# DeepMETv2/DeepMETv2

Measured on AMD Instinct MI355X. Metric: events/sec (4.5k PF cands, k=16), higher is better.
Workload: dtype f32

## Files before the change

deepmetv2_amd/csrc/knn.hip:

```cpp
#include <stdlib.h>

#include "common.h"
#include "knn_common.h"
#include "knn_key64.h"
#include "nls_body.h"

namespace dmet {
namespace {

constexpr int kTileC = 32;
constexpr int kQMax = 8;
constexpr int kMaxSplit = 8;
constexpr int kWavesPerGroup = 4;

#define DMET_PKSUB_LO " op_sel:[0,0] op_sel_hi:[0,1] neg_lo:[0,1] neg_hi:[0,1]\n\t"
#define DMET_PKSUB_HI " op_sel:[1,0] op_sel_hi:[1,1] neg_lo:[0,1] neg_hi:[0,1]\n\t"
__device__ __forceinline__ void pk_dist_step4(f2 &accA, f2 &accB, f2 vxy, f2 vzw, f2 wxy, f2 wzw, f2 q0, f2 q1, f2 q2,
                                              f2 q3)
{
    f2 t0, t1, t2, t3;
    asm("v_pk_add_f32 %[t0], %[vxy], %[q0]" DMET_PKSUB_LO
        "v_pk_add_f32 %[t1], %[wxy], %[q0]" DMET_PKSUB_LO
        "v_pk_add_f32 %[t2], %[vxy], %[q1]" DMET_PKSUB_HI
        "v_pk_add_f32 %[t3], %[wxy], %[q1]" DMET_PKSUB_HI
// ... 105 lines not shown
        for (int p = 0; p < KP; p += 4) {
            *reinterpret_cast<float4 *>(ld + p) = make_float4(d[p], d[p + 1], d[p + 2], d[p + 3]);
            *reinterpret_cast<int4 *>(lj + p) = make_int4(j[p], j[p + 1], j[p + 2], j[p + 3]);
        }
    }
    return d[KP - 1];
}

#ifdef DMET_KNN_STAMP
__device__ unsigned long long g_knn_stamps[1 << 16][4];
#endif

#ifndef DMET_F2_MIN_NODES
#define DMET_F2_MIN_NODES 800
#endif
constexpr int kF2MinNodes = DMET_F2_MIN_NODES;
constexpr int kFilterMaxSplit = 2;
#ifndef DMET_F2_SPLIT_MIN_NODES
#define DMET_F2_SPLIT_MIN_NODES 2560
#endif
constexpr int kF2SplitMinNodes = DMET_F2_SPLIT_MIN_NODES;
constexpr int kF2MaxNodes = 65536;

struct KnnPlan {
    int total_tiles;
    int n_full;
    int split;
    int form1_events;
};

struct KnnArgs {
    const float *x;
    const int64_t *ptr;
    int B;
    int64_t N;
    int D, k;
    int32_t *nbr;
    float *dist;
    uint16_t *nbr16;
    float *wsd;
    int32_t *wsj;
    const KnnPlan *plan;
    const int32_t *order;
    const int32_t *tile_ptr;
    float *psd;
    int32_t *psj;
    const int32_t *flags;
    int flag_min;
    const int32_t *any;
    const int32_t *qlist;
    const int32_t *pos_of;
    int requery_groups;
    int requery_tile_queries;
};

__device__ __forceinline__ uint16_t local_id16(int32_t j, int ev_lo)
{
    return (uint16_t)(j >= 0 ? (unsigned)(j - ev_lo) : 0xFFFFu);
}

constexpr int kMaxSortedEvents = 4096;

struct KnnPlanOut {
    int tile_queries, simds, max_split;
    int32_t *order, *pos_of, *tile_ptr;
    KnnPlan *plan;
};

__device__ __forceinline__ int xcd_dealt_position(int rank, int B)
{
    if (B < 4 * kNumXcd) return rank;
    const int c = rank % (2 * kNumXcd), g = rank / (2 * kNumXcd);
    const int bin = c < kNumXcd ? c : 2 * kNumXcd - 1 - c;
    const int idx = 2 * g + (c >= kNumXcd ? 1 : 0);
    const int rem = B % (2 * kNumXcd), full = B / (2 * kNumXcd);
    int start = 0;
    for (int b = 0; b < bin; ++b)
        start += 2 * full + (b < min(rem, kNumXcd) ? 1 : 0) + ((rem > kNumXcd && b > 2 * kNumXcd - 1 - rem) ? 1 : 0);
    return start + idx;
}

template <bool XY = false>
__device__ __forceinline__ void knn_plan_body(const int64_t *__restrict__ ptr, int B, const KnnPlanOut &o,
                                              const int64_t *__restrict__ cptr = nullptr)
{
    const int tile_queries = o.tile_queries, simds = o.simds, max_split = o.max_split;
    int32_t *__restrict__ order = o.order, *__restrict__ pos_of = o.pos_of, *__restrict__ tile_ptr = o.tile_ptr;
    KnnPlan *__restrict__ plan = o.plan;
    __shared__ int part[256];
    const int tid = threadIdx.x;
    if (B <= kMaxSortedEvents) {
        for (int b = tid; b < B; b += 256) {
            const int64_t nb = ptr[b + 1] - ptr[b];
            int rank = 0;
            if constexpr (XY) {
                const int64_t xb = nb > 0 ? cptr[b + 1] - cptr[b] : -1;
                for (int c = 0; c < B; ++c) {
                    const int64_t nc = ptr[c + 1] - ptr[c];
                    const int64_t xc = nc > 0 ? cptr[c + 1] - cptr[c] : -1;
                    rank += (xc > xb || (xc == xb && (nc > nb || (nc == nb && c < b)))) ? 1 : 0;
                }
            } else {
                for (int c = 0; c < B; ++c) {
                    const int64_t nc = ptr[c + 1] - ptr[c];
                    rank += (nc > nb || (nc == nb && c < b)) ? 1 : 0;
                }
// ... 110 lines not shown
    int lo = 0, hi = B;
    while (hi - lo > 1) {
        const int mid = (lo + hi) >> 1;
        if (tile_ptr[mid] <= t) lo = mid; else hi = mid;
    }
    return lo;
}

template <int DP, bool EXACT_D, int NLD>
__device__ __forceinline__ void load_tile(float4 (&pf)[NLD], const float *__restrict__ x, int D, int c0, int cntc,
                                          int lane)
{
    const float inf = __builtin_inff();
    if (EXACT_D) {
        const float4 *g = reinterpret_cast<const float4 *>(x + (int64_t)c0 * DP);
        const int n4 = cntc * (DP / 4);
#pragma unroll
        for (int m = 0; m < NLD; ++m) {
            const int idx = lane + m * kWave;
            pf[m] = (idx < n4) ? g[idx] : make_float4(inf, inf, inf, inf);
        }
    } else {
#pragma unroll
        for (int m = 0; m < NLD; ++m) {
            float v[4];
#pragma unroll
            for (int e = 0; e < 4; ++e) {
                const int flat = (lane + m * kWave) * 4 + e;
                const int c = flat / DP, dd = flat - c * DP;
                v[e] = (c < cntc) ? ((dd < D) ? x[(int64_t)(c0 + c) * D + dd] : 0.0f) : inf;
            }
            pf[m] = make_float4(v[0], v[1], v[2], v[3]);
        }
    }
}

__device__ __forceinline__ float chain_dist32(const float *__restrict__ xj, const float (&q)[32])
{
    const float4 *g = reinterpret_cast<const float4 *>(xj);
    float acc = 0.0f;
#pragma unroll
    for (int c = 0; c < 8; ++c) {
        const float4 v = g[c];
        float df;
        df = v.x - q[4 * c + 0]; acc = __builtin_fmaf(df, df, acc);
        df = v.y - q[4 * c + 1]; acc = __builtin_fmaf(df, df, acc);
        df = v.z - q[4 * c + 2]; acc = __builtin_fmaf(df, df, acc);
        df = v.w - q[4 * c + 3]; acc = __builtin_fmaf(df, df, acc);
    }
    return acc;
}

constexpr int kRequeryMax = 8;
constexpr int kRequeryGroups = 512;

__device__ __forceinline__ unsigned long long requery_word(float d, int j)
{
    return d < kKnnSentinel ? (((unsigned long long)__float_as_uint(d) << 32) | (unsigned)j) : ~0ull;
}

__device__ __forceinline__ void knn_requery_body(const KnnArgs &a, float *__restrict__ cache, const int cache_floats,
                                                 unsigned long long *__restrict__ red, const int group, const int ngroups)
{
    const int tid = threadIdx.x, wv = tid >> 6, lane = tid & 63;
    const int64_t nf64 = *a.any;
    const int nflag = (int)(nf64 < a.N ? nf64 : a.N);
    const int k = a.k;
    for (int it = group; it < nflag; it += ngroups) {
        const int q = a.qlist[it];
        int lo = 0, hi = a.B;
        while (hi - lo > 1) {
            const int mid = (lo + hi) >> 1;
            if (a.ptr[mid] <= q) lo = mid; else hi = mid;
        }
        const int ev = lo;
        const int ev_lo = (int)a.ptr[ev], ev_hi = (int)a.ptr[ev + 1];
        const int n = ev_hi - ev_lo;
        const int xt = a.tile_ptr[a.pos_of[ev]] + (q - ev_lo) / a.requery_tile_queries;
        if (a.flags[xt] > kRequeryMax) continue;
        const bool cached = n <= cache_floats;
        float qrow[32];
        {
            const float4 *g = reinterpret_cast<const float4 *>(a.x + (int64_t)q * 32);
#pragma unroll
            for (int c = 0; c < 8; ++c) {
                const float4 v = g[c];
                qrow[4 * c] = v.x; qrow[4 * c + 1] = v.y; qrow[4 * c + 2] = v.z; qrow[4 * c + 3] = v.w;
            }
        }
        __syncthreads();
        if (cached) {
            for (int j0 = tid; j0 < n; j0 += 4 * 256) {
                float4 r[4][8];
#pragma unroll
                for (int u = 0; u < 4; ++u) {
                    const float4 *g = reinterpret_cast<const float4 *>(a.x + (int64_t)(ev_lo + min(j0 + 256 * u, n - 1)) * 32);
#pragma unroll
                    for (int c = 0; c < 8; ++c) r[u][c] = g[c];
                }
#pragma unroll
                for (int u = 0; u < 4; ++u) {
                    float dc = 0.0f;
#pragma unroll
                    for (int c = 0; c < 8; ++c) {
                        float df;
                        df = r[u][c].x - qrow[4 * c + 0]; dc = __builtin_fmaf(df, df, dc);
                        df = r[u][c].y - qrow[4 * c + 1]; dc = __builtin_fmaf(df, df, dc);
                        df = r[u][c].z - qrow[4 * c + 2]; dc = __builtin_fmaf(df, df, dc);
                        df = r[u][c].w - qrow[4 * c + 3]; dc = __builtin_fmaf(df, df, dc);
                    }
                    if (j0 + 256 * u < n) cache[j0 + 256 * u] = dc;
                }
            }
            __syncthreads();
        }
        unsigned long long last = 0ull;
        bool first = true;
        for (int r = 0; r < k; ++r) {
            unsigned long long best = ~0ull;
            for (int j = tid; j < n; j += 256) {
                const float d = cached ? cache[j] : chain_dist32(a.x + (int64_t)(ev_lo + j) * 32, qrow);
                const unsigned long long w = requery_word(d, ev_lo + j);
                if ((first || w > last) && w < best) best = w;
            }
#pragma unroll
            for (int off = 32; off > 0; off >>= 1) {
                const unsigned long long o = __shfl_xor(best, off, 64);
                if (o < best) best = o;
            }
            if (lane == 0) red[wv] = best;
            __syncthreads();
            best = red[0];
#pragma unroll
            for (int w = 1; w < 4; ++w) if (red[w] < best) best = red[w];
            __syncthreads();
            const bool found = best != ~0ull;
            if (tid == 0) {
                const int bj = found ? (int)(unsigned)best : -1;
                a.nbr[(int64_t)q * k + r] = bj;
                if (a.nbr16) a.nbr16[(int64_t)q * k + r] = local_id16(bj, ev_lo);
                a.dist[(int64_t)q * k + r] = found ? __uint_as_float((unsigned)(best >> 32)) : kKnnSentinel;
            }
            if (!found) {
                if (tid == 0)
                    for (int rr = r + 1; rr < k; ++rr) {
                        a.nbr[(int64_t)q * k + rr] = -1;
                        a.dist[(int64_t)q * k + rr] = kKnnSentinel;
                        if (a.nbr16) a.nbr16[(int64_t)q * k + rr] = 0xFFFFu;
                    }
                break;
            }
            last = best;
            first = false;
        }
    }
}

template <int DP, int KP, int TQ, bool EXACT_D, typename... Per>
__global__ __launch_bounds__(kWave * kWavesPerGroup, 3) void knn_kernel(const KnnArgs a, Per... per_arg)
{
    constexpr bool PER = pack_has<RadPeriod, Per...>, XY = pack_has<KnnQuerySet, Per...>;
    static_assert(!PER || TQ == 2, "the periodic sweep is the packed two-query form (D <= 8)");
    const RadPeriod per = rad_periods(per_arg...);
    __shared__ KnnShared<DP, TQ> sh_all[kWavesPerGroup];
    const int wv_ = __builtin_amdgcn_readfirstlane(threadIdx.x >> 6);
    KnnShared<DP, TQ> &sh = sh_all[wv_];
    int first_group = 0;
    if constexpr (DP == 32 && !XY) {
        if (a.qlist) {
            if (a.any && *a.any == 0) return;
            if ((int)blockIdx.x < a.requery_groups) {
                constexpr int kFloats = (int)((sizeof(sh_all) - 64) / sizeof(float));
                knn_requery_body(a, reinterpret_cast<float *>(sh_all), kFloats,
                                 reinterpret_cast<unsigned long long *>(reinterpret_cast<char *>(sh_all) + sizeof(sh_all) - 64),
                                 (int)blockIdx.x, a.requery_groups);
                return;
            }
            first_group = a.requery_groups;
        }
    }
    const int item = ((int)blockIdx.x - first_group) * kWavesPerGroup + wv_;
    const int lane = threadIdx.x & 63;
#ifdef DMET_KNN_STAMP
    if (lane == 0 && item < (1 << 16)) {
        g_knn_stamps[item][0] = __builtin_amdgcn_s_memrealtime();
        unsigned hwid, xcc;
        asm volatile("s_getreg_b32 %0, hwreg(HW_REG_HW_ID)" : "=s"(hwid));
        asm volatile("s_getreg_b32 %0, hwreg(HW_REG_XCC_ID)" : "=s"(xcc));
        g_knn_stamps[item][2] = hwid;
        g_knn_stamps[item][3] = xcc;
        g_knn_stamps[item][1] = 0;
    }
#endif
    const float *__restrict__ x = a.x;
    const int64_t *__restrict__ ptr = a.ptr;
    const KnnQuerySet qs = query_set(a.x, a.ptr, per_arg...);
    const float *__restrict__ qx = qs.qx;
    const int64_t *__restrict__ qptr = qs.qptr;
    const int D = a.D;
    constexpr int QT = kWave * TQ;

    const int n_full = a.plan->n_full, split = a.plan->split, total = a.plan->total_tiles;
    int tile = item, sub = 0, nsub = 1;
    if (item >= n_full && !a.flags) {
        const int r = item - n_full;
        tile = n_full + r / split;
        sub = r % split;
        nsub = split;
    }
    if (tile >= total) return;
    if (a.any && *a.any == 0) return;
    if (a.flags && a.flags[tile] < a.flag_min) return;
    const int pos = find_tile_event(a.tile_ptr, a.B, tile);
    const int ev = a.order[pos];
    const int ev_lo = (int)qptr[ev], ev_hi = (int)qptr[ev + 1];
    const int q_first = ev_lo + (tile - a.tile_ptr[pos]) * QT;

    int clo = XY ? (int)ptr[ev] : ev_lo, chi = XY ? (int)ptr[ev + 1] : ev_hi;
    if (nsub > 1) {
        const int chunk = (((chi - clo) + nsub - 1) / nsub + 1) & ~1;
        clo = min(chi, clo + sub * chunk);
        chi = min(chi, clo + chunk);
    }

    int qi[TQ];
    bool valid[TQ];
    float tau[TQ];
    int cnt[TQ];
    float *ld[TQ];
    int32_t *lj[TQ];
    f2 q2[(TQ == 2) ? DP : 1];
    float q1[(TQ == 1) ? DP : 1];
#pragma unroll
    for (int t = 0; t < TQ; ++t) {
        qi[t] = q_first + t * kWave + lane;
// ... 78 lines not shown
                    df = v.z - q1[4 * c4 + 2]; accA = __builtin_fmaf(df, df, accA);
                    df = w.z - q1[4 * c4 + 2]; accB = __builtin_fmaf(df, df, accB);
                    df = v.w - q1[4 * c4 + 3]; accA = __builtin_fmaf(df, df, accA);
                    df = w.w - q1[4 * c4 + 3]; accB = __builtin_fmaf(df, df, accB);
                }
                dA[0] = accA; dB[0] = accB;
            }
#pragma unroll
            for (int t = 0; t < TQ; ++t) {
#pragma unroll
                for (int u = 0; u < 2; ++u) {
                    const float dj = u ? dB[t] : dA[t];
                    bool pass = dj < tau[t];
#ifdef DMET_KNN_NOSELECT
                    pass = pass && (dj < -1.0f);
#endif
                    if (pass) {
                        sh.queue[t][cnt[t]][lane] = make_uint2(__float_as_uint(dj), (unsigned)(c0 + cc + u));
                        cnt[t]++;
                    }
                }
                if (__any(cnt[t] > kQMax - 2)) {
                    tau[t] = drain_queue<KP>(sh.queue[t], lane, cnt[t], (fresh >> t) & 1u, valid[t], ld[t], lj[t]);
                    if (!valid[t]) tau[t] = -1.0f;
                    cnt[t] = 0;
                    fresh &= ~(1u << t);
                }
            }
        }
    }
#ifdef DMET_KNN_STAMP
    if (lane == 0 && item < (1 << 16)) g_knn_stamps[item][1] = __builtin_amdgcn_s_memrealtime();
#endif
#pragma unroll
    for (int t = 0; t < TQ; ++t) {
        (void)drain_queue<KP>(sh.queue[t], lane, cnt[t], (fresh >> t) & 1u, valid[t], ld[t], lj[t]);
        if (valid[t] && nsub == 1) {
            const int64_t qq = qi[t];
            if (a.k == KP) {
#pragma unroll
                for (int p = 0; p < KP; p += 4) {
                    *reinterpret_cast<float4 *>(a.dist + qq * KP + p) = *reinterpret_cast<const float4 *>(ld[t] + p);
                    *reinterpret_cast<int4 *>(a.nbr + qq * KP + p) = *reinterpret_cast<const int4 *>(lj[t] + p);
                }
            } else {
                for (int p = 0; p < a.k; ++p) {
                    a.dist[qq * a.k + p] = ld[t][p];
                    a.nbr[qq * a.k + p] = lj[t][p];
                }
            }
            if (a.nbr16)
                for (int p = 0; p < a.k; ++p) a.nbr16[qq * a.k + p] = local_id16(lj[t][p], ev_lo);
        }
    }
}

template <int KP, typename... Qs>
__global__ __launch_bounds__(256) void knn_merge_kernel(const KnnArgs a, int tile_queries, Qs... qs_arg)
{
    if (a.any && *a.any == 0) return;
    const int n_full = a.plan->n_full, split = a.plan->split, total = a.plan->total_tiles;
    if (split <= 1) return;
    const int64_t slot = (int64_t)blockIdx.x * blockDim.x + threadIdx.x;
    const int tile = n_full + (int)(slot / tile_queries);
    if (tile >= total) return;
    if (a.flags && a.flags[tile] < a.flag_min) return;
    const int pos = find_tile_event(a.tile_ptr, a.B, tile);
    const int ev = a.order[pos];
    const int64_t *__restrict__ qptr = query_set(a.x, a.ptr, qs_arg...).qptr;
    const int64_t qi = qptr[ev] + (int64_t)(tile - a.tile_ptr[pos]) * tile_queries + (slot % tile_queries);
    if (qi >= qptr[ev + 1]) return;
    const float *pd = a.psd + slot * split * KP;
    const int32_t *pj = a.psj + slot * split * KP;
    int head[kMaxSplit];
#pragma unroll
    for (int s = 0; s < kMaxSplit; ++s) head[s] = 0;
    for (int p = 0; p < a.k; ++p) {
        float bd = kKnnSentinel;
        int32_t bj = -1;
        int bs = -1;
#pragma unroll
        for (int s = 0; s < kMaxSplit; ++s) {
            if (s < split && head[s] < KP) {
                const float d = pd[s * KP + head[s]];
                const int32_t j = pj[s * KP + head[s]];
                if (j >= 0 && (bs < 0 || d < bd || (d == bd && j < bj))) { bd = d; bj = j; bs = s; }
            }
        }
#pragma unroll
        for (int s = 0; s < kMaxSplit; ++s) head[s] += (s == bs) ? 1 : 0;
        a.dist[qi * a.k + p] = bd;
        a.nbr[qi * a.k + p] = bj;
        if (a.nbr16) a.nbr16[qi * a.k + p] = local_id16(bj, (int)a.ptr[ev]);
    }
}

#include "knn_filter.h"

int num_simds()
{
    static int cached = 0;
    if (cached == 0) {
        int dev = 0, cus = 0;
        if (hipGetDevice(&dev) == hipSuccess &&
            hipDeviceGetAttribute(&cus, hipDeviceAttributeMultiprocessorCount, dev) == hipSuccess && cus > 0)
            cached = cus * 4;
// ... 78 lines not shown
    w.pos_of = reinterpret_cast<int32_t *>(take(sizeof(int32_t) * ((size_t)B + 1)));
    w.tile_ptr = reinterpret_cast<int32_t *>(take(sizeof(int32_t) * ((size_t)B + 1)));
    w.wsd = reinterpret_cast<float *>(take(sizeof(float) * (size_t)N * KP));
    w.wsj = reinterpret_cast<int32_t *>(take(sizeof(int32_t) * (size_t)N * KP));
    w.psd = reinterpret_cast<float *>(take(sizeof(float) * ps_elems));
    w.psj = reinterpret_cast<int32_t *>(take(sizeof(int32_t) * ps_elems));
    if (!exact_only) {
        w.fplan = reinterpret_cast<KnnPlan *>(take(sizeof(KnnPlan)));
        w.forder = reinterpret_cast<int32_t *>(take(sizeof(int32_t) * ((size_t)B + 1)));
        w.fpos_of = reinterpret_cast<int32_t *>(take(sizeof(int32_t) * ((size_t)B + 1)));
        w.ftile_ptr = reinterpret_cast<int32_t *>(take(sizeof(int32_t) * ((size_t)B + 1)));
        w.nrm = reinterpret_cast<float *>(take(sizeof(float) * (size_t)N));
        w.nrec = (N >> 5) + B + 1;
        w.rec = reinterpret_cast<uint8_t *>(take((size_t)w.nrec * kRecBytesMax));
        w.zero_bytes = sizeof(int32_t) * ((size_t)exact_tiles_max(N, B) + 4) + (size_t)N;
        w.flags = reinterpret_cast<int32_t *>(take(w.zero_bytes));
        w.any = w.flags + exact_tiles_max(N, B);
        w.qflag = reinterpret_cast<uint8_t *>(w.any + 4);
        w.qlist = reinterpret_cast<int32_t *>(take(sizeof(int32_t) * (size_t)N));
    }
    w.bytes = (size_t)(p - reinterpret_cast<uintptr_t>(ws));
    return w;
}

inline int filter_mode()
{
    const char *e = getenv("DMET_KNN_PATH");
    if (e && strcmp(e, "exact") == 0) return 0;
#if defined(DMET_KNN_EXPERIMENT) || defined(DMET_FILTER_ABL) || defined(DMET_F2_ABL) || defined(DMET_F2_SAMEREC)
    if (e && strcmp(e, "filter_only") == 0) return 2;
#endif
    return 1;
}

inline int filter_form2()
{
    const char *e = getenv("DMET_KNN_FILTER");
    return (e && strcmp(e, "1") == 0) ? 0 : 1;
}

constexpr float kF2CutScale = 1.25f;
inline float knn_cut_scale()
{
    const char *e = getenv("DMET_KNN_CUT");
    if (!e || !*e) return kF2CutScale;
    if (strcmp(e, "0") == 0 || strcmp(e, "off") == 0) return -1.0f;
    char *end = nullptr;
    const float v = strtof(e, &end);
    return (end != e && *end == '\0' && v >= 0.0f && v <= 1e6f) ? v : kF2CutScale;
}

inline int knn_run_cut() { return env_is("DMET_KNN_RUNCUT", "0") ? 0 : 1; }

template <int KF, int NH = 1>
int launch_filter(const KnnFilterArgs &f, const KnnWorkspace &w, int simds, const KnnPlanOut &px, const KnnPlanOut &pf,
                  hipStream_t st, const KnnRider *rider, const BnAffine *affine)
{
    const int slots = simds * kF2WavesPerSimd;
    if (affine) {
        if constexpr (NH == 1)
            hipLaunchKernelGGL((knn_prep_kernel<1, true>), dim3((unsigned)((w.nrec * kWave + 255) / 256 + 2)), dim3(256), 0, st, f.x,
                               f.ptr, f.B, f.N, w.nrm, w.rec, w.nrec, reinterpret_cast<uint32_t *>(w.flags), w.zero_bytes, px,
                               pf, f.form2, *affine, 0);
    } else {
        hipLaunchKernelGGL((knn_prep_kernel<NH>), dim3((unsigned)((w.nrec * kWave + 255) / 256 + 2)), dim3(256), 0, st, f.x,
                           f.ptr, f.B, f.N, w.nrm, w.rec, w.nrec, reinterpret_cast<uint32_t *>(w.flags), w.zero_bytes, px, pf,
                           f.form2, BnAffine{}, 0);
    }
    DMET_LAUNCH_CHECK("knn_prep_kernel");
    const int64_t ftiles_max = (f.N + kFQ - 1) / kFQ + f.B;
    const int64_t fblocks = (ftiles_max + slots + kWavesPerGroup - 1) / kWavesPerGroup;
    if (f.form2) {
        KnnFilterArgs fr = f;
        int64_t grid = fblocks;
        if (rider) {
            fr.rW = rider->W; fr.rb = rider->b; fr.rP = rider->P; fr.rQ = rider->Q; fr.r_sliced = rider->sliced;
            fr.first_rider = (int)fblocks;
            grid = fblocks + rider_groups();
        }
        hipLaunchKernelGGL((knn_filter12_kernel<KF, NH>), dim3((unsigned)grid), dim3(kWave * kWavesPerGroup), 0, st, fr);
        DMET_LAUNCH_CHECK("knn_filter12_kernel");
    } else {
        if constexpr (NH == 1) hipLaunchKernelGGL((knn_filter_kernel<KF>), dim3((unsigned)fblocks), dim3(kWave * kWavesPerGroup), 0, st, f);
        DMET_LAUNCH_CHECK("knn_filter_kernel");
    }
    constexpr int kRerankQpb = 4 * (kWave / filter_list_len(KF));
    constexpr int kRerankParts = (kFQ + kRerankQpb - 1) / kRerankQpb;
    const int64_t tail_max = ftiles_max < slots ? ftiles_max : slots;
    if constexpr (NH == 1) {
        if (f.no_rerank) return 0;
        hipLaunchKernelGGL((knn_rerank_kernel<KF>), dim3((unsigned)(tail_max * kRerankParts)), dim3(256), 0, st, f);
        DMET_LAUNCH_CHECK("knn_rerank_kernel");
    }
    return 0;
}

template <int DP, int KP, int TQ>
void launch_sweep(int64_t blocks, unsigned dyn, hipStream_t st, const KnnArgs &a, bool exact_d, const RadPeriod *per,
                  const KnnQuerySet *qs)
{
    const dim3 grid((unsigned)blocks), block(kWave * kWavesPerGroup);
    with_pack<DP <= 8, true>(per, qs, [&](auto... pack) {
        if (exact_d) hipLaunchKernelGGL((knn_kernel<DP, KP, TQ, true, decltype(pack)...>), grid, block, dyn, st, a, pack...);
        else hipLaunchKernelGGL((knn_kernel<DP, KP, TQ, false, decltype(pack)...>), grid, block, dyn, st, a, pack...);
    });
}

template <int KP>
void launch_merge(int64_t slots, hipStream_t st, const KnnArgs &a, int tile_queries, const KnnQuerySet *qs)
{
    with_pack<false, true>(nullptr, qs, [&](auto... pack) {
        hipLaunchKernelGGL((knn_merge_kernel<KP, decltype(pack)...>), dim3((unsigned)((slots + 255) / 256)), dim3(256), 0, st, a,
                           tile_queries, pack...);
    });
}

template <int DP, int KP>
KnnOutcome launch_knn(const KnnBuild &r, const KnnWorkspace &w)
{
    KnnOutcome done;
    constexpr int TQ = (DP <= 32) ? 2 : 1;
    constexpr int QT = kWave * TQ;
    const KnnQuerySet *qs = r.qs.qx ? &r.qs : nullptr;
    int simds = num_simds();
    if (simds > kMaxSimds) simds = kMaxSimds;
    bool use_filter = false;
    if constexpr ((DP == 32 || DP == 64) && KP <= 32)
        use_filter = !qs && r.D == DP && r.k <= 20 && aligned16(r.x) && filter_mode() != 0 && (DP == 32 || filter_form2());
    constexpr int NH = DP == 64 ? 2 : 1;
    const int slots = simds * kF2WavesPerSimd;
    const KnnPlanOut px{QT, simds, kMaxSplit, w.order, w.pos_of, w.tile_ptr, w.plan};
    const KnnPlanOut pf{kFQ, slots, kFilterMaxSplit, w.forder, w.fpos_of, w.ftile_ptr, w.fplan};
    if (qs) {
        hipLaunchKernelGGL(knn_plan_xy_kernel, dim3(1), dim3(256), 0, r.st, qs->qptr, r.ptr, r.B, px);
        DMET_LAUNCH_CHECK("knn_plan_xy_kernel");
    } else if (!use_filter) {
        hipLaunchKernelGGL(knn_plan_kernel, dim3(1), dim3(256), 0, r.st, r.ptr, r.B, px, pf);
        DMET_LAUNCH_CHECK("knn_plan_kernel");
    }
    KnnArgs a{r.x, r.ptr, r.B, r.N, r.D, r.k, r.nbr, r.dist, r.nbr16, w.wsd, w.wsj, w.plan, w.order, w.tile_ptr, w.psd, w.psj,
              nullptr, 0, nullptr, nullptr, nullptr, 0, QT};
    if (!qs && !use_filter && hipMemsetAsync(w.flags, 0, w.zero_bytes, r.st) != hipSuccess)
        return hip_fail(hipGetLastError(), "hipMemsetAsync");

    if (use_filter) {
        KnnFilterArgs f{r.x, r.ptr, r.B, r.N, r.k, w.nrm, w.rec, w.fplan, w.forder, w.fpos_of, w.ftile_ptr,
                        w.psd, w.psj, r.nbr, r.dist, r.nbr16, w.flags, w.any, w.qflag, w.qlist, w.tile_ptr, QT, filter_form2(),
                        NH == 1 ? 1.0f : 1.5f, nullptr, nullptr, nullptr, nullptr, 0, 0,
                        (aligned16(r.nbr) && aligned16(r.dist) && aligned16(r.nbr16) && !env_is("DMET_KNN_EMIT", "lanes")) ? 1 : 0, 0,
                        knn_cut_scale(), w.any + 1, knn_run_cut()};
        f.no_rerank = (f.form2 && r.hint.min_nodes >= kF2MinNodes && r.hint.max_nodes >= r.hint.min_nodes &&
                       r.hint.max_nodes <= kF2MaxNodes) ? 1 : 0;
        const BnAffine *affine = (NH == 1 && r.affine.raw) ? &r.affine : nullptr;
        const KnnRider *rider = (NH == 1 && f.form2 && r.rider.P) ? &r.rider : nullptr;
        int rc = 0;
        if constexpr (DP == 32 || DP == 64) {
            if constexpr (KP == 8) rc = launch_filter<8, NH>(f, w, simds, px, pf, r.st, rider, affine);
            else if constexpr (KP == 16) rc = launch_filter<16, NH>(f, w, simds, px, pf, r.st, rider, affine);
            else if constexpr (KP == 32) rc = launch_filter<20, NH>(f, w, simds, px, pf, r.st, rider, affine);
        }
        if (rc) return rc;
        done.affine_done = affine != nullptr;
        done.rider_done = rider != nullptr;
        if (filter_mode() == 2) return done;
        a.flags = w.flags;
        a.any = w.any;
        if constexpr (NH == 1) {
            a.qlist = w.qlist;
            a.pos_of = w.pos_of;
            a.requery_groups = kRequeryGroups;
            a.flag_min = kRequeryMax + 1;
        } else {
            a.flag_min = 1;
        }
    }

    const int64_t tiles_max = (r.N + QT - 1) / QT + r.B;
    const int64_t blocks = (tiles_max + simds + kWavesPerGroup - 1) / kWavesPerGroup + a.requery_groups;
    unsigned dyn = 0;
#ifdef DMET_KNN_EXPERIMENT
    if (const char *e = getenv("DMET_KNN_EXTRA_LDS")) dyn = (unsigned)atoi(e);
#endif
    const bool exact_d = r.D == DP && aligned16(r.x) && (!qs || aligned16(qs->qx));
    launch_sweep<DP, KP, TQ>(blocks, dyn, r.st, a, exact_d, r.per, qs);
    DMET_LAUNCH_CHECK(qs ? "knn_kernel (two sets)" : "knn_kernel");
    if (!use_filter) {
        int64_t mslots = (int64_t)simds * QT;
        if (tiles_max * QT < mslots) mslots = tiles_max * QT;
        launch_merge<KP>(mslots, r.st, a, QT, qs);
        DMET_LAUNCH_CHECK(qs ? "knn_merge_kernel (two sets)" : "knn_merge_kernel");
    }
    return done;
}

template <int DP>
KnnOutcome dispatch_k(const KnnBuild &r)
{
    const KnnWorkspace w = carve_workspace(r.ws, r.N, r.B, padded_k(r.k), r.qs.qx != nullptr);
    if (r.k <= 8) return launch_knn<DP, 8>(r, w);
    if (r.k <= 16) return launch_knn<DP, 16>(r, w);
    if (r.k <= 32) return launch_knn<DP, 32>(r, w);
    return launch_knn<DP, 64>(r, w);
}

KnnOutcome knn_build(const KnnBuild &r)
{
    if (r.D <= 4) return dispatch_k<4>(r);
    if (r.D <= 8) return dispatch_k<8>(r);
    if (r.D <= 16) return dispatch_k<16>(r);
    if (r.D <= 32) return dispatch_k<32>(r);
    return dispatch_k<64>(r);
}

}
}

using namespace dmet;

static thread_local KnnSizeHint g_size_hint;

extern "C" int dmet_knn_size_hint(int min_nodes, int max_nodes)
{
    DMET_REQUIRE(min_nodes >= 0 && max_nodes >= 0, "dmet_knn_size_hint: negative size");
    g_size_hint.min_nodes = min_nodes;
    g_size_hint.max_nodes = max_nodes;
    return 0;
}

static KnnSizeHint take_size_hint()
{
    const KnnSizeHint h = g_size_hint;
// ... 202 lines not shown
```

deepmetv2_amd/csrc/knn_filter.h:

```cpp
constexpr int kFQ = 64;

typedef float f32x16 __attribute__((ext_vector_type(16)));
typedef short bf16x8 __attribute__((ext_vector_type(8)));
typedef _Float16 f16x8 __attribute__((ext_vector_type(8)));

struct KnnFilterArgs {
    const float *x;
    const int64_t *ptr;
    int B;
    int64_t N;
    int k;
    float *nrm;
    uint8_t *rec;
    const KnnPlan *plan;
    const int32_t *order;
    const int32_t *pos_of;
    const int32_t *tile_ptr;
    float *psd;
    int32_t *psj;
    int32_t *nbr;
    float *dist;
    uint16_t *nbr16;
    int32_t *flags;
    int32_t *any;
    uint8_t *qflag;
    int32_t *qlist;
    const int32_t *xtile_ptr;
    int xtile_queries;
    int form2;
    float slack_scale;
    const float *rW, *rb;
    float *rP, *rQ;
    int r_sliced;
    int first_rider;
    int emit_coalesced;
    int no_rerank;
    float cut_scale;
    int32_t *retries;
    int run_cut;
};

struct KnnRider {
    const float *W = nullptr, *b = nullptr;
    float *P = nullptr, *Q = nullptr;
    int sliced = 0;
};

static_assert(sizeof(BnAffine) == 48 && alignof(BnAffine) == 8,
              "BnAffine + the padded kernarg_pad are the 56-byte tail of knn_prep_kernel's argument block: keep its size");

inline int rider_groups()
{
    static int cached = 0;
    if (cached == 0) {
        const char *e = getenv("DMET_KNN_RIDER_GROUPS");
        const int v = e ? atoi(e) : 0;
        cached = (v >= 1 && v <= 4096) ? v : 512;
    }
    return cached;
}

__device__ __forceinline__ void flag_query(const KnnFilterArgs &a, int q, int xtile)
{
    a.qflag[q] = 1;
    atomicAdd(a.flags + xtile, 1);
    const int slot = atomicAdd(a.any, 1);
    if (slot < a.N) a.qlist[slot] = q;
}

__device__ __forceinline__ unsigned bf16_rne_bits(float f)
{
    const unsigned u = __float_as_uint(f);
    return (u + 0x7fffu + ((u >> 16) & 1u)) >> 16;
}

constexpr int kRecFragBytes = 4 * kWave * 16;
constexpr int rec_bytes(int NH) { return kRecFragBytes * NH + 32 * 4; }
constexpr int kRecBytes = rec_bytes(1);
constexpr int kRecBytesMax = rec_bytes(2);

__device__ __forceinline__ int64_t rec_base_tile(const int64_t *__restrict__ ptr, int b) { return (ptr[b] >> 5) + b; }

constexpr int kRec16FragBytes = 2 * kWave * 16;
constexpr float kF16WideLimit = 16384.0f;
static_assert(kRec16FragBytes + kWave * 16 <= rec_bytes(1) && 2 * kRec16FragBytes + kWave * 16 <= rec_bytes(2),
              "the fold fragment fits the record");
constexpr float kF2NormP[4] = {0x1p15f, 0x1p5f, 0x1p-6f, 0x1p-17f};
constexpr float kF2NormInvP[4] = {0x1p-15f, 0x1p-5f, 0x1p6f, 0x1p17f};
constexpr float kF2NormMax = 65504.0f * 0x1p15f;
constexpr float kF2TauC[2] = {0x1p14f, 0x1p-15f};
constexpr float kF2TauRepMax = 65504.0f * 0x1p14f;

__device__ __forceinline__ bool f2_in_domain64(int64_t n) { return n >= kF2MinNodes && n <= kF2MaxNodes; }
// ... 890 lines not shown
}

template <int KP, int NH = 1>
__device__ __forceinline__ void filter2_wave(const KnnFilterArgs &a, F2Wave &S, int *tickets, int group, int wv, int lane)
{
    constexpr int M = f2_list_len(KP);
    static_assert(f2_list_cap(M) == KP, "f2_running_tau reads slot KP - 1 of the list");
    constexpr int D = 32 * NH;
    constexpr int MS = (M + 1 + 3) & ~3;
    const int col = lane & 31, hh = lane >> 5;
    const uint8_t *__restrict__ rec = a.rec;
    const int64_t *__restrict__ ptr = a.ptr;

    const int n_full = a.plan->n_full, split = a.plan->split, total = a.plan->total_tiles;
    const int item = group * kWavesPerGroup + wv;
    int tile = item, sub = 0, nsub = 1;
    if (item >= n_full) {
        const int r = item - n_full;
        tile = n_full + r / split;
        sub = r % split;
        nsub = split;
    }
    if (tile >= total) return;
    const int pos = find_tile_event(a.tile_ptr, a.B, tile);
    const int ev = a.order[pos];
    const int ev_lo = (int)ptr[ev], ev_hi = (int)ptr[ev + 1];
    const int q_first = ev_lo + (tile - a.tile_ptr[pos]) * kFQ;
    if (!f2_in_domain(ev_hi - ev_lo)) {
        if (NH != 1 && sub == 0) {
            const int q = q_first + lane;
            if (q < ev_hi) {
                flag_query(a, q, a.xtile_ptr[pos] + (q - ev_lo) / a.xtile_queries);
            }
        }
        return;
    }
    int clo = ev_lo, chi = ev_hi;
    if (nsub > 1) {
        if (ev_hi - ev_lo < kF2SplitMinNodes) {
            if (sub != 0) return;
            nsub = 1;
        } else {
            const int chunk = (((chi - clo) + nsub - 1) / nsub + 31) & ~31;
            clo = min(chi, clo + sub * chunk);
            chi = min(chi, clo + chunk);
        }
    }
    const int64_t rbase = (ptr[ev] >> 5) + ev;
    const int64_t rlast = rbase + (ev_hi - ev_lo - 1) / 32;
    const int t_lo = (clo - ev_lo) / 32, t_hi = (chi - ev_lo + 31) / 32;

    const int myq = q_first + hh * 32 + col;
    const bool valid = myq < ev_hi;
    float t_fix = -__builtin_inff();
    bool act = valid;
    for (int attempt = 0;; ++attempt) {
    F2Lane<M> L;
#pragma unroll
    for (int p = 0; p < M; ++p) L.tk[p] = kKnnSentinel;
    L.tau = attempt == 0 ? -__builtin_inff() : t_fix;
    L.margin = __builtin_inff();
    L.tq = 0u;
    L.rep = 0.0f;
    L.cnt = 0;
    L.overflow = false;
    {
        f16x8 bq[2][2 * NH];
#pragma unroll
        for (int b = 0; b < 2; ++b) {
            const int64_t qrec = min(rbase + (q_first - ev_lo) / 32 + b, rlast);
            const f16x8 *g = reinterpret_cast<const f16x8 *>(rec + qrec * rec_bytes(NH));
#pragma unroll
            for (int m = 0; m < 2 * NH; ++m) bq[b][m] = g[m * 64 + lane] * (_Float16)-2.0f;
        }
        if (attempt == 0) {
            const int t_def = min(t_hi, t_lo + kF2Defer);
            f2_sweep<M, true, false, NH>(L, S, rec, rbase, t_lo, t_def, bq, lane, hh, valid);
            if (a.run_cut && a.cut_scale >= 0.0f && a.k == KP && t_def < t_hi) {
                const float tkk = L.tk[KP - 1];
                int qi = valid ? myq : ev_lo;
                asm volatile("" : "+v"(qi));
                const float m = f2_cut<NH>(tkk, a.nrm[qi], a.cut_scale) - tkk;
                if (tkk < kKnnSentinel && m > 0.0f && m < __builtin_inff()) L.margin = __builtin_fmaf(m, 0.01f, m);
                L.tau = fminf(L.tau, tkk + L.margin);
            }
            f2_sweep<M, true, true, NH>(L, S, rec, rbase, t_def, t_hi, bq, lane, hh, valid);
            if (a.cut_scale >= 0.0f) {
                float tkk = kKnnSentinel;
#pragma unroll
                for (int p = 0; p < KP; ++p)
                    if (p == a.k - 1) tkk = L.tk[p];
                if (tkk < kKnnSentinel) {
                    int qi = valid ? myq : ev_lo;
                    asm volatile("" : "+v"(qi));
                    const float cut = f2_cut<NH>(tkk, a.nrm[qi], a.cut_scale);
                    L.tau = fminf(L.tau, cut);
                }
            }
            f2_sweep<M, false, true, NH>(L, S, rec, rbase, t_lo, t_def, bq, lane, hh, valid);
        } else {
            f2_sweep<M, false, true, NH>(L, S, rec, rbase, t_lo, t_hi, bq, lane, hh, valid);
        }
    }
    f2_compact<M>(L, S, lane, kF2Slots);
#if defined(DMET_F2_ABL) && DMET_F2_ABL >= 1
    return;
#endif

    const int64_t qrow_id = valid ? myq : ev_lo;
    float qrow[D];
    {
        const float4 *g = reinterpret_cast<const float4 *>(a.x + qrow_id * D);
#pragma unroll
        for (int c = 0; c < D / 4; ++c) {
            const float4 v = g[c];
            qrow[4 * c] = v.x; qrow[4 * c + 1] = v.y; qrow[4 * c + 2] = v.z; qrow[4 * c + 3] = v.w;
        }
    }
    static_assert(__builtin_bit_cast(unsigned, kKnnSentinel) == kKey64SentinelBits, "knn_key64.h clamps to the sentinel");
    double kk[KP];
#pragma unroll
    for (int p = 0; p < KP; ++p) kk[p] = key64_as_double(kKey64Empty);
    const int nent = (act && !L.overflow) ? L.cnt : 0;
    int slot = 0;
    unsigned cmask = 0u;
    int ctile = 0;
    uint2 enext = S.ent[0][lane];
    auto pop = [&]() __attribute__((always_inline)) -> int32_t {
        const bool take = cmask == 0u && slot < nent;
        cmask = take ? enext.x : cmask;
        ctile = take ? (int)(enext.y & kF2TileMask) : ctile;
        slot += take ? 1 : 0;
        enext = S.ent[min(slot, kF2Slots - 1)][lane];
        int32_t jl = -1;
        if (cmask != 0u) {
            const int r = __builtin_clz(cmask);
            cmask &= ~(0x80000000u >> r);
            jl = ctile * 32 + f2_mask_row(r);
        }
        return jl;
    };
    const float4 *x4 = reinterpret_cast<const float4 *>(a.x);
#ifdef DMET_RR_PRIO
    __builtin_amdgcn_s_setprio(DMET_RR_PRIO);
#endif
    if constexpr (NH != 1) {
        for (;;) {
            const int32_t jl = pop();
            if (!__any(jl >= 0)) break;
            const int32_t j = ev_lo + jl;
            const float4 *row = x4 + (int64_t)(jl >= 0 ? j : ev_lo) * (D / 4);
            float4 v[D / 4];
#pragma unroll
            for (int c = 0; c < D / 4; ++c) v[c] = row[c];
            float dc = 0.0f;
#pragma unroll
            for (int c = 0; c < D / 4; ++c) {
                float df;
                df = v[c].x - qrow[4 * c + 0]; dc = __builtin_fmaf(df, df, dc);
                df = v[c].y - qrow[4 * c + 1]; dc = __builtin_fmaf(df, df, dc);
                df = v[c].z - qrow[4 * c + 2]; dc = __builtin_fmaf(df, df, dc);
                df = v[c].w - qrow[4 * c + 3]; dc = __builtin_fmaf(df, df, dc);
            }
            key64_insert<KP>(kk, key64_word(__float_as_uint(dc), (unsigned)j, jl >= 0));
        }
    } else {
    struct HalfRows { float4 v0, v1, v2, v3, v4, v5, v6, v7; };
#ifdef DMET_RR_FULLROW
    auto fetch = [&](int32_t jl) __attribute__((always_inline)) -> HalfRows {
        const int32_t jc = ev_lo + (jl >= 0 ? jl : 0);
        const int64_t o = lane & 7;
        const int sub = lane >> 3;
        HalfRows R;
        R.v0 = x4[(int64_t)__shfl(jc, 0 + sub, 64) * 8 + o];
        R.v1 = x4[(int64_t)__shfl(jc, 8 + sub, 64) * 8 + o];
        R.v2 = x4[(int64_t)__shfl(jc, 16 + sub, 64) * 8 + o];
        R.v3 = x4[(int64_t)__shfl(jc, 24 + sub, 64) * 8 + o];
        R.v4 = x4[(int64_t)__shfl(jc, 32 + sub, 64) * 8 + o];
        R.v5 = x4[(int64_t)__shfl(jc, 40 + sub, 64) * 8 + o];
        R.v6 = x4[(int64_t)__shfl(jc, 48 + sub, 64) * 8 + o];
        R.v7 = x4[(int64_t)__shfl(jc, 56 + sub, 64) * 8 + o];
        return R;
    };
#else
    const uint64_t xb = reinterpret_cast<uint64_t>(a.x + (int64_t)ev_lo * D);
    const uint64_t xbs = ((uint64_t)(unsigned)__builtin_amdgcn_readfirstlane((int)(xb >> 32)) << 32) |
                         (unsigned)__builtin_amdgcn_readfirstlane((int)xb);
    typedef float f32x4 __attribute__((ext_vector_type(4)));
    typedef const f32x4 __attribute__((address_space(1))) *GlobalRow;
    auto ld = [](GlobalRow g, int i) __attribute__((always_inline)) -> float4 {
        const f32x4 v = g[i];
        return make_float4(v.x, v.y, v.z, v.w);
    };
    auto fetch = [&](int32_t jl) __attribute__((always_inline)) -> HalfRows {
        const int32_t jc = jl >= 0 ? jl : 0;
// ... 442 lines not shown
```

Baseline: 51360.

## Make exact kNN fallback a persistent grid-stride walk over flagged tiles

Splits the kNN kernel body into a per-item device function and adds a WALK variant. In that variant a capped, persistent grid of groups strides over all tiles and processes only those whose flag reaches the threshold, replacing a launch of one group per tile. The default requery group count drops from 512 to 256, and the tile groups are sized at three per CU. It also adds an optional priority-dephasing scheme for the filter kernel, which is off by default. The aim is to avoid launching and retiring many groups that exit immediately on unflagged tiles, at the cost of less parallelism when many tiles are flagged.

Result: no change. 51380, median of 3 (+0.0%).

```diff
diff --git a/deepmetv2_amd/csrc/knn.hip b/deepmetv2_amd/csrc/knn.hip
--- a/deepmetv2_amd/csrc/knn.hip
+++ b/deepmetv2_amd/csrc/knn.hip
@@ -181,6 +181,7 @@
     const int32_t *pos_of;
     int requery_groups;
     int requery_tile_queries;
+    int tile_groups;
 };
 
 __device__ __forceinline__ uint16_t local_id16(int32_t j, int ev_lo)
@@ -397,7 +398,6 @@
 }
 
 constexpr int kRequeryMax = 8;
-constexpr int kRequeryGroups = 512;
 
 __device__ __forceinline__ unsigned long long requery_word(float d, int j)
 {
@@ -502,30 +502,11 @@
 }
 
 template <int DP, int KP, int TQ, bool EXACT_D, typename... Per>
-__global__ __launch_bounds__(kWave * kWavesPerGroup, 3) void knn_kernel(const KnnArgs a, Per... per_arg)
+__device__ __forceinline__ void knn_item(const KnnArgs &a, KnnShared<DP, TQ> &sh, const int item, const int lane, Per... per_arg)
 {
     constexpr bool PER = pack_has<RadPeriod, Per...>, XY = pack_has<KnnQuerySet, Per...>;
     static_assert(!PER || TQ == 2, "the periodic sweep is the packed two-query form (D <= 8)");
     const RadPeriod per = rad_periods(per_arg...);
-    __shared__ KnnShared<DP, TQ> sh_all[kWavesPerGroup];
-    const int wv_ = __builtin_amdgcn_readfirstlane(threadIdx.x >> 6);
-    KnnShared<DP, TQ> &sh = sh_all[wv_];
-    int first_group = 0;
-    if constexpr (DP == 32 && !XY) {
-        if (a.qlist) {
-            if (a.any && *a.any == 0) return;
-            if ((int)blockIdx.x < a.requery_groups) {
-                constexpr int kFloats = (int)((sizeof(sh_all) - 64) / sizeof(float));
-                knn_requery_body(a, reinterpret_cast<float *>(sh_all), kFloats,
-                                 reinterpret_cast<unsigned long long *>(reinterpret_cast<char *>(sh_all) + sizeof(sh_all) - 64),
-                                 (int)blockIdx.x, a.requery_groups);
-                return;
-            }
-            first_group = a.requery_groups;
-        }
-    }
-    const int item = ((int)blockIdx.x - first_group) * kWavesPerGroup + wv_;
-    const int lane = threadIdx.x & 63;
 #ifdef DMET_KNN_STAMP
     if (lane == 0 && item < (1 << 16)) {
         g_knn_stamps[item][0] = __builtin_amdgcn_s_memrealtime();
@@ -710,6 +691,40 @@
             if (a.nbr16)
                 for (int p = 0; p < a.k; ++p) a.nbr16[qq * a.k + p] = local_id16(lj[t][p], ev_lo);
         }
+    }
+}
+
+template <int DP, int KP, int TQ, bool EXACT_D, bool WALK, typename... Per>
+__global__ __launch_bounds__(kWave * kWavesPerGroup, 3) void knn_kernel(const KnnArgs a, Per... per_arg)
+{
+    constexpr bool XY = pack_has<KnnQuerySet, Per...>;
+    static_assert(!WALK || ((DP == 32 || DP == 64) && sizeof...(Per) == 0), "the filter's fallback only");
+    __shared__ KnnShared<DP, TQ> sh_all[kWavesPerGroup];
+    const int wv_ = __builtin_amdgcn_readfirstlane(threadIdx.x >> 6);
+    KnnShared<DP, TQ> &sh = sh_all[wv_];
+    int first_group = 0;
+    if constexpr (DP == 32 && !XY) {
+        if (a.qlist) {
+            if (a.any && *a.any == 0) return;
+            if ((int)blockIdx.x < a.requery_groups) {
+                constexpr int kFloats = (int)((sizeof(sh_all) - 64) / sizeof(float));
+                knn_requery_body(a, reinterpret_cast<float *>(sh_all), kFloats,
+                                 reinterpret_cast<unsigned long long *>(reinterpret_cast<char *>(sh_all) + sizeof(sh_all) - 64),
+                                 (int)blockIdx.x, a.requery_groups);
+                return;
+            }
+            first_group = a.requery_groups;
+        }
+    }
+    const int item = ((int)blockIdx.x - first_group) * kWavesPerGroup + wv_;
+    const int lane = threadIdx.x & 63;
+    if constexpr (WALK) {
+        if (*a.any == 0) return;
+        const int total = a.plan->total_tiles;
+        for (int it = item; it < total; it += a.tile_groups * kWavesPerGroup)
+            if (a.flags[it] >= a.flag_min) knn_item<DP, KP, TQ, EXACT_D>(a, sh, it, lane);
+    } else {
+        knn_item<DP, KP, TQ, EXACT_D>(a, sh, item, lane, per_arg...);
     }
 }
 
@@ -894,6 +909,36 @@
 
 inline int knn_run_cut() { return env_is("DMET_KNN_RUNCUT", "0") ? 0 : 1; }
 
+constexpr int kF2Dephase = 0;
+inline int knn_dephase()
+{
+    const char *e = getenv("DMET_KNN_DEPHASE");
+    if (!e || !*e) return kF2Dephase;
+    if (strcmp(e, "0") == 0) return 0;
+    if ((e[0] == 'h' || e[0] == 'p') && e[1] >= '1' && e[1] <= '3' && e[2] == '\0') return (e[1] - '0') + (e[0] == 'p' ? 4 : 0);
+    return kF2Dephase;
+}
+
+inline int knn_resident_groups(int simds)
+{
+    if (const char *e = getenv("DMET_KNN_DEPHASE_RESIDENT")) {
+        const int v = atoi(e);
+        if (v >= 2 && v <= 65536) return v;
+    }
+    return simds / 4 * 2;
+}
+
+constexpr int kExactGroupsPerCu = 3;
+constexpr int kFallbackQueryGroups = 256;
+inline int knn_fallback_cap()
+{
+    if (const char *e = getenv("DMET_KNN_FALLBACK_GROUPS")) {
+        const int v = atoi(e);
+        if (v >= 1 && v <= 4096) return v;
+    }
+    return 0;
+}
+
 template <int KF, int NH = 1>
 int launch_filter(const KnnFilterArgs &f, const KnnWorkspace &w, int simds, const KnnPlanOut &px, const KnnPlanOut &pf,
                   hipStream_t st, const KnnRider *rider, const BnAffine *affine)
@@ -942,9 +987,15 @@
                   const KnnQuerySet *qs)
 {
     const dim3 grid((unsigned)blocks), block(kWave * kWavesPerGroup);
+    if constexpr ((DP == 32 || DP == 64) && KP <= 32) {
+        if (a.tile_groups > 0) {
+            hipLaunchKernelGGL((knn_kernel<DP, KP, TQ, true, true>), grid, block, dyn, st, a);
+            return;
+        }
+    }
     with_pack<DP <= 8, true>(per, qs, [&](auto... pack) {
-        if (exact_d) hipLaunchKernelGGL((knn_kernel<DP, KP, TQ, true, decltype(pack)...>), grid, block, dyn, st, a, pack...);
-        else hipLaunchKernelGGL((knn_kernel<DP, KP, TQ, false, decltype(pack)...>), grid, block, dyn, st, a, pack...);
+        if (exact_d) hipLaunchKernelGGL((knn_kernel<DP, KP, TQ, true, false, decltype(pack)...>), grid, block, dyn, st, a, pack...);
+        else hipLaunchKernelGGL((knn_kernel<DP, KP, TQ, false, false, decltype(pack)...>), grid, block, dyn, st, a, pack...);
     });
 }
 
@@ -981,7 +1032,7 @@
         DMET_LAUNCH_CHECK("knn_plan_kernel");
     }
     KnnArgs a{r.x, r.ptr, r.B, r.N, r.D, r.k, r.nbr, r.dist, r.nbr16, w.wsd, w.wsj, w.plan, w.order, w.tile_ptr, w.psd, w.psj,
-              nullptr, 0, nullptr, nullptr, nullptr, 0, QT};
+              nullptr, 0, nullptr, nullptr, nullptr, 0, QT, 0};
     if (!qs && !use_filter && hipMemsetAsync(w.flags, 0, w.zero_bytes, r.st) != hipSuccess)
         return hip_fail(hipGetLastError(), "hipMemsetAsync");
 
@@ -990,7 +1041,7 @@
                         w.psd, w.psj, r.nbr, r.dist, r.nbr16, w.flags, w.any, w.qflag, w.qlist, w.tile_ptr, QT, filter_form2(),
                         NH == 1 ? 1.0f : 1.5f, nullptr, nullptr, nullptr, nullptr, 0, 0,
                         (aligned16(r.nbr) && aligned16(r.dist) && aligned16(r.nbr16) && !env_is("DMET_KNN_EMIT", "lanes")) ? 1 : 0, 0,
-                        knn_cut_scale(), w.any + 1, knn_run_cut()};
+                        knn_cut_scale(), w.any + 1, knn_run_cut(), knn_dephase(), knn_resident_groups(simds)};
         f.no_rerank = (f.form2 && r.hint.min_nodes >= kF2MinNodes && r.hint.max_nodes >= r.hint.min_nodes &&
                        r.hint.max_nodes <= kF2MaxNodes) ? 1 : 0;
         const BnAffine *affine = (NH == 1 && r.affine.raw) ? &r.affine : nullptr;
@@ -1007,18 +1058,27 @@
         if (filter_mode() == 2) return done;
         a.flags = w.flags;
         a.any = w.any;
+        const int cap = knn_fallback_cap();
         if constexpr (NH == 1) {
             a.qlist = w.qlist;
             a.pos_of = w.pos_of;
-            a.requery_groups = kRequeryGroups;
+            a.requery_groups = cap ? (cap / 2 > 0 ? cap / 2 : 1) : kFallbackQueryGroups;
             a.flag_min = kRequeryMax + 1;
         } else {
             a.flag_min = 1;
         }
+        const int grid = cap ? cap : simds / 4 * kExactGroupsPerCu;
+        a.tile_groups = grid - a.requery_groups > 0 ? grid - a.requery_groups : 1;
     }
 
     const int64_t tiles_max = (r.N + QT - 1) / QT + r.B;
-    const int64_t blocks = (tiles_max + simds + kWavesPerGroup - 1) / kWavesPerGroup + a.requery_groups;
+    int64_t blocks = (tiles_max + simds + kWavesPerGroup - 1) / kWavesPerGroup;
+    if (a.tile_groups > 0) {
+        const int64_t one_each = (tiles_max + kWavesPerGroup - 1) / kWavesPerGroup;
+        if (a.tile_groups > one_each) a.tile_groups = (int)one_each;
+        blocks = a.tile_groups;
+    }
+    blocks += a.requery_groups;
     unsigned dyn = 0;
 #ifdef DMET_KNN_EXPERIMENT
     if (const char *e = getenv("DMET_KNN_EXTRA_LDS")) dyn = (unsigned)atoi(e);
diff --git a/deepmetv2_amd/csrc/knn_filter.h b/deepmetv2_amd/csrc/knn_filter.h
--- a/deepmetv2_amd/csrc/knn_filter.h
+++ b/deepmetv2_amd/csrc/knn_filter.h
@@ -38,7 +38,24 @@
     float cut_scale;
     int32_t *retries;
     int run_cut;
+    int dephase;
+    int resident_groups;
 };
+
+__device__ __forceinline__ int f2_dephase_level(const KnnFilterArgs &a)
+{
+    const int g = (int)blockIdx.x;
+    if (a.dephase == 0 || g >= a.resident_groups) return 0;
+    const int cls = (a.dephase & 4) ? (g & 1) : (g >= (a.resident_groups >> 1) ? 1 : 0);
+    return cls ? (a.dephase & 3) : 0;
+}
+
+__device__ __forceinline__ void f2_raise_prio(int level)
+{
+    if (level == 1) __builtin_amdgcn_s_setprio(1);
+    else if (level == 2) __builtin_amdgcn_s_setprio(2);
+    else if (level == 3) __builtin_amdgcn_s_setprio(3);
+}
 
 struct KnnRider {
     const float *W = nullptr, *b = nullptr;
@@ -1035,6 +1052,7 @@
 
     const int myq = q_first + hh * 32 + col;
     const bool valid = myq < ev_hi;
+    f2_raise_prio(f2_dephase_level(a));
     float t_fix = -__builtin_inff();
     bool act = valid;
     for (int attempt = 0;; ++attempt) {
@@ -1124,6 +1142,7 @@
         return jl;
     };
     const float4 *x4 = reinterpret_cast<const float4 *>(a.x);
+    if (a.dephase != 0) __builtin_amdgcn_s_setprio(0);
 #ifdef DMET_RR_PRIO
     __builtin_amdgcn_s_setprio(DMET_RR_PRIO);
 #endif
```
